# indianajohn/akaze-rust

Measured on AMD Instinct MI355X. Metric: Mpix/s through extract_features (4 oct x 4 sub), higher is better.
Workload: dtype f32

## Files before the change

### akaze-rust_amd/csrc/akz_api.cpp

```cpp
#include "akz_ctx.hpp"

unsigned akz::host_cpu_share() {
    unsigned n = std::max(1u, std::thread::hardware_concurrency());
    cpu_set_t set;
    if (sched_getaffinity(0, sizeof(set), &set) == 0) n = std::max(1, CPU_COUNT(&set));
    if (FILE* f = fopen("/sys/fs/cgroup/cpu.max", "r")) {
        char q[32] = {0};
        long period = 0;
        if (fscanf(f, "%31s %ld", q, &period) == 2 && period > 0 && strcmp(q, "max") != 0)
            n = std::min<unsigned>(n, (unsigned)std::max(1L, atol(q) / period));
        fclose(f);
    }
    if (const char* e = std::getenv("LOCAL_WORLD_SIZE")) {
        const int ranks = atoi(e);
        if (ranks > 1) n = std::max(2u, n / (unsigned)ranks);
    }
    return std::max(1u, n);
}

int level_info_out(const std::vector<LevelPlan>& plan, uint64_t level, double* etime, double* esigma,
                          uint32_t* octave, uint32_t* sublevel, uint32_t* sigma_size, uint32_t* lw, uint32_t* lh,
                          uint32_t* det_sigma, uint64_t* n_tau, double* tau, uint64_t tau_cap) {
    if (level >= plan.size()) {
        set_error("level out of range");
// ... 390 lines not shown
}
int akz_ctx_set_match_mode(akz_ctx* c, int mode) {
    AKZ_TRY(bind(c));
    if (mode < 0 || mode > 3) return AKZ_ERR_INVALID_ARG;
    c->match_mode = mode;
    for (akz_ctx* l : c->lanes) l->match_mode = mode;
    return AKZ_OK;
}
int akz_ctx_set_fed_mode(akz_ctx* c, int mode) {
    AKZ_TRY(bind(c));
    if (mode != 0 && mode != 2) return AKZ_ERR_INVALID_ARG;
    c->fed_mode = mode;
    for (akz_ctx* l : c->lanes) l->fed_mode = mode;
    return AKZ_OK;
}
const char* akz_fed_kernel_name(void) { return "k_level_march + k_fed_own"; }
int akz_debug_march_bands(int kind, uint32_t w, uint32_t h, uint32_t n, int half_width, int32_t* rows, uint32_t cap,
                          uint32_t* n_bands) {
    if (!n_bands || (cap && !rows) || kind < 0 || kind > 1 || w < 16 || h < 16 || n == 0 || half_width < 1 || half_width > 4)
        return AKZ_ERR_INVALID_ARG;
    *n_bands = launch::march_band_rows(kind, w, h, n, half_width, rows, cap);
    return AKZ_OK;
}
const char* akz_detector_kernel_name(void) { return "detector (k_detector_march + k_detector_tiled)"; }
int akz_debug_set_schedule(akz_ctx* c, int key, int value) {
    if (!c || key < 0 || key > 10) return AKZ_ERR_INVALID_ARG;
    AKZ_TRY(bind(c));
    c->sched[key] = value;
    if (key == 7 || key == 8) launch::march_min_band_rows(c->sched[7], c->sched[8]);
    if (key == 4) {
        c->big_px_sync = value > 0 ? (uint64_t)value * 1000u : gates::kBigPxSync;
        c->big_px_async = value > 0 ? (uint64_t)value * 1000u : gates::kBigPxAsync;
        c->lane_px = value > 0 ? (uint64_t)value * 1000u : gates::kLanePx;
        for (akz_ctx* l : c->lanes) {
            l->big_px_sync = std::max(c->big_px_sync, c->lane_px);
            l->big_px_async = std::max(c->big_px_async, c->lane_px);
        }
    }
    return AKZ_OK;
}
int akz_debug_placement_verdict(float spin_pair_ms, float tiny_pair_ms, float tiny_alone_ms, float spin_ms) {
    return akz::placement_verdict(spin_pair_ms, tiny_pair_ms, tiny_alone_ms, spin_ms);
}
int akz_debug_stream_placement(akz_ctx* c, int* info) {
    if (!c || !info) return AKZ_ERR_INVALID_ARG;
    AKZ_TRY(bind(c));
    info[0] = c->placed ? 1 : 0;
    info[1] = c->pre_mode;
    info[2] = c->place_replaced;
    info[3] = c->place_collisions + c->lane_collisions;
    return AKZ_OK;
}
// ... 86 lines not shown
```

### akaze-rust_amd/csrc/akz_ctx.hpp

```cpp
#pragma once
#include <algorithm>
#include <cmath>
#include <cstdlib>
#include <cstddef>
#include <cstring>
#include <atomic>
#include <condition_variable>
#include <functional>
#include <map>
#include <memory>
#include <mutex>
#include <thread>
#include <sched.h>
#include <time.h>
#include <type_traits>

#include "akz_internal.hpp"
#include "akz_select.hpp"
#include "akz_pool.hpp"
#include "akz_gates.hpp"

#define AKZ_LOCAL __attribute__((visibility("hidden")))

namespace akz {
// ... 103 lines not shown
    std::atomic<uint32_t> cand_cap_hint{1u << 15};
    std::atomic<int> live_results{0};
    bool dead = false;
    std::atomic<uint32_t> last_total_cands{0};
    std::atomic<uint64_t> last_cand_shape{0};
    hipStream_t aux = nullptr;
    std::mutex aux_m;
    hipStream_t coarse = nullptr;
    hipStream_t pre = nullptr;
    hipEvent_t pre_done = nullptr;
    hipStream_t copy = nullptr;
    DevBuf stage[kSlots];
    hipEvent_t staged[kSlots] = {nullptr, nullptr, nullptr};
    std::vector<akz_ctx*> lanes;
    unsigned next_lane = 0;
    bool is_lane = false;
    bool eager_finish = true;
    std::shared_ptr<Finisher> fin;
    hipEvent_t lane_in = nullptr;
    uint64_t stream_min_px = gates::kStreamPx;
    int prep_mode = 2;
    int det_mode = 2;
    int fed_mode = 2;
    int sched[11] = {0, 1, 0, 0, 0, 0, 0, 0, 0, 0, 0};
    uint64_t big_px = gates::kBigPxAsync;
    uint64_t big_px_sync = gates::kBigPxSync, big_px_async = gates::kBigPxAsync;
    uint64_t lane_px = gates::kLanePx;
    static constexpr uint64_t kLaunchMarchPx = gates::kMarchPx;
    uint64_t launch_min_px = kLaunchMarchPx;
    bool placed = false;
    int pre_mode = 0;
    int place_replaced = 0;
    int place_collisions = 0;
    int place_retries = 0;
    int lane_collisions = 0;
    hipEvent_t probe_ev[2] = {nullptr, nullptr};
    int profiling = 0;
    akz_profile prof{};
    struct Span { int stage; hipEvent_t a, b; int row; };
    std::vector<Span> spans;
    std::vector<akz_kernel_row> rows;
    std::vector<hipEvent_t> ev_pool;
    std::mutex ev_m;
    static constexpr int kFedRing = 4;
    hipEvent_t fed_ev[kFedRing] = {nullptr, nullptr, nullptr, nullptr};
    hipEvent_t pre_ev[kFedRing] = {nullptr, nullptr, nullptr, nullptr};
    std::atomic<uint64_t> begin_seq{0};
// ... 238 lines not shown
```

### akaze-rust_amd/csrc/akz_extract_begin.cpp

```cpp
#include "akz_extract.hpp"

namespace {
enum class Prep : uint8_t {
    Tiled,
    Stream,
    LevelMarch,
    Resident
};
enum class Det : uint8_t {
    Fallback,
    NmsFused,
    TiledSet,
    March
};
struct BeginRoute {
    bool big = false;
    int prep_mode = 0;
    int pre_on = 0;
    bool level1_clone = false;
    size_t res_first = 0;
    size_t fork_level = 0;
    size_t oct1 = 0;
    bool own_kernels = true;
    struct Level {
// ... 244 lines not shown
    StageTimer st(c, AKZ_ST_FED);
    st.kernel(AKZ_KR_FED_OWN, n_tau, lv.w, lv.h, n, fed_num_launches(c, n_tau, lv.w, lv.h, n), 0, (uint64_t)lv.w * lv.h * n * n_tau);
    AKZ_TRY(fed_impl(c, fed_in, A, B, b.P(i, AKZ_LFLOW), b.keep_all ? b.P(i, AKZ_LSTEP) : nullptr, lv.w, lv.h, n, lv.tau.data(), n_tau,
                     ride ? &np : nullptr, &rode));
    b.prepared[i + 1] = rode ? 1 : 0;
    return AKZ_OK;
}

int run_levels(BeginState& b, size_t lo, size_t hi) {
    akz_ctx* c = b.c;
    const std::vector<LevelPlan>& plan = b.r->plan;
    for (size_t i = lo; i < hi; ++i) {
        if (i >= 2) interleave_detector(b, i - 1);
        if (i == b.rt.res_first) return resident_tail(b, i);
        float* A = b.P(i, AKZ_LT);
        const bool on_coarse = i >= b.rt.fork_level;
        if (on_coarse) AKZ_TRY(ensure(c, c->scratch_coarse, plane_bytes(plan[b.rt.fork_level].w, plan[b.rt.fork_level].h, b.n)));
        float* B = (float*)(on_coarse ? c->scratch_coarse.p : c->scratch[5].p);
        AKZ_TRY(b.rt.lv[i].prep == Prep::LevelMarch ? level_by_march(b, i, A, B) : level_by_launches(b, i, A, B));
    }
    return AKZ_OK;
}

int detectors(BeginState& b, size_t lo, size_t hi, hipStream_t on) {
    akz_ctx* c = b.c;
    const akz_config& cfg = b.r->cfg;
    const uint32_t n = b.n;
    std::map<uint32_t, std::vector<launch::DetLevelDesc>> sets;
    for (size_t l = lo; l < hi; ++l) {
        if (b.det_done[l]) continue;
        const LevelPlan& lv = b.r->plan[l];
        const float thr = (float)cfg.detector_threshold, bm = border_margin(lv, cfg);
        if (b.rt.lv[l].det == Det::TiledSet) {
            sets[lv.det_sigma].push_back(launch::DetLevelDesc{b.P(l, AKZ_LSMOOTH), b.P(l, AKZ_LX), b.P(l, AKZ_LY), b.P(l, AKZ_LXX),
                                                             b.P(l, AKZ_LYY), b.P(l, AKZ_LXY), b.P(l, AKZ_LDET), lv.w, lv.h, (uint32_t)l, bm});
            continue;
        }
        if (detector_one_pass(b, l, on)) continue;
        {
            StageTimer st(c, AKZ_ST_DETECTOR);
            AKZ_TRY(detector_impl(c, b.P(l, AKZ_LSMOOTH), lv.det_sigma, b.P(l, AKZ_LX), b.P(l, AKZ_LY), b.P(l, AKZ_LXX),
                                  b.P(l, AKZ_LYY), b.P(l, AKZ_LXY), b.P(l, AKZ_LDET), lv.w, lv.h, n));
        }
        StageTimer st(c, AKZ_ST_NMS);
        launch::nms(on, b.P(l, AKZ_LDET), lv.w, lv.h, n, (uint64_t)lv.w * lv.h, (uint32_t)l, thr, bm, b.d_cand, b.cap, b.d_count);
    }
    for (auto& kv : sets) {
        const uint32_t maxn = launch::detector_tiled_set_max();
        for (size_t i = 0; i < kv.second.size(); i += maxn) {
            StageTimer st(c, AKZ_ST_DETECTOR, on);
            if (c->profiling) {
                c->prof.det_launches += 1;
                uint64_t set_px = 0;
                for (size_t j = i; j < std::min(kv.second.size(), i + maxn); ++j) set_px += (uint64_t)kv.second[j].w * kv.second[j].h * n;
                c->prof.det_px += set_px;
                st.kernel(AKZ_KR_DETECTOR_TILED, kv.first, kv.second[i].w, kv.second[i].h, n, 1, set_px);
            }
            launch::detector_tiled_set(on, kv.first, kv.second.data() + i, (uint32_t)std::min<size_t>(maxn, kv.second.size() - i),
                                       n, (float)cfg.detector_threshold, b.d_cand, b.cap, b.d_count);
        }
    }
    return AKZ_OK;
}

int fork_and_join(BeginState& b, hipStream_t* done_on) {
    akz_ctx* c = b.c;
    hipStream_t s = b.s;
    if (!c->coarse) AKZ_HIP_TRY(hipStreamCreateWithFlags(&c->coarse, hipStreamNonBlocking));
// ... 120 lines not shown
```

### akaze-rust_amd/csrc/akz_internal.hpp

```cpp
#pragma once
#include <hip/hip_runtime.h>

#include <cstdint>
#include <functional>
#include <string>
#include <vector>

#include "../../include/akaze_hip.h"
#include "../../include/akaze_hip_debug.h"

namespace akz {

void set_error(const std::string& msg);
unsigned host_cpu_share();

using TrialsOnDevice = std::function<int(const float*, const float*, const float*, const float*, uint32_t, const uint32_t*, uint32_t,
                                         float, float, float*, int32_t*)>;
int remove_outliers_impl(const akz_keypoint* keypoints_0, uint64_t n0, const akz_keypoint* keypoints_1, uint64_t n1,
                         const akz_match* matches, uint64_t n_matches, uint64_t num_trials, float epsilon_model,
                         float epsilon_inlier, akz_match* out, uint64_t* n_out, const TrialsOnDevice& trials_on_device);

#define AKZ_HIP_TRY(expr)                                                                          \
    do {                                                                                           \
        hipError_t _e = (expr);                                                                    \
// ... 163 lines not shown
                          float* lyy, float* lxy, float* ldet_out, uint32_t w, uint32_t h, uint32_t n, uint32_t level,
                          float thr, float border_m, Candidate* d_cand, uint32_t cap, uint32_t* d_count);
bool blur5_stream_supported(uint32_t w, uint32_t h, uint32_t ntaps, bool is_u8);
void blur5_stream_u8(hipStream_t s, const uint8_t* in, float* out, uint32_t w, uint32_t h, uint32_t n, const float* k);
void blur5_stream_f32(hipStream_t s, const float* in, float* out, uint32_t w, uint32_t h, uint32_t n, const float* k);
uint32_t march_band_rows(int kind, uint32_t w, uint32_t h, uint32_t n, int S, int32_t* cs_ce, uint32_t cap);
bool blur5_march_supported(uint32_t w, uint32_t h, uint32_t ntaps);
void blur5_march_u8(hipStream_t s, const uint8_t* in, float* out, uint32_t w, uint32_t h, uint32_t n, const float* k);
void blur5_march_f32(hipStream_t s, const float* in, float* out, uint32_t w, uint32_t h, uint32_t n, const float* k);
bool contrast_march_supported(uint32_t w, uint32_t h, uint32_t ntaps, uint32_t nbins);
void contrast_march(hipStream_t s, const float* in, uint32_t w, uint32_t h, uint32_t n, const float* g3,
                    unsigned long long* d_hmax_bits, uint32_t nbins, uint32_t* d_hist, double* d_thr);
void contrast_thresholds(hipStream_t s, const unsigned long long* d_hmax_bits, uint32_t nbins, uint32_t n, double* d_thr);
bool contrast_stream_supported(uint32_t w, uint32_t h, uint32_t ntaps, uint32_t nbins);
void contrast_stream(hipStream_t s, const float* in, uint32_t w, uint32_t h, uint32_t n, const float* g3,
                     unsigned long long* d_hmax_bits, uint32_t nbins, uint32_t* d_hist, double* d_thr);
bool prep_stream_supported(uint32_t w, uint32_t h);
void prep_stream(hipStream_t s, const float* prev, bool half, float* lt_out, float* lsmooth, float* lflow, uint32_t w,
                 uint32_t h, uint32_t pw, uint32_t ph, uint32_t n, const float* g3, const double* d_k, uint32_t k_pow);
bool detector_march_supported(uint32_t sigma, uint32_t w, uint32_t h, float border_m, bool nms);
void detector_march(hipStream_t s, const float* lsmooth, uint32_t sigma, float* lx, float* ly, float* lxx, float* lyy,
                    float* lxy, float* ldet_out, uint32_t w, uint32_t h, uint32_t n, uint32_t level, float thr,
                    float border_m, Candidate* d_cand, uint32_t cap, uint32_t* d_count);
bool head_fused_supported(uint32_t w, uint32_t h, uint32_t ntaps0, uint32_t ntaps1);
void head_fused_u8(hipStream_t s, const uint8_t* in, float* lt0, float* blurred, float* gx, float* gy, uint32_t w, uint32_t h, uint32_t n,
                   const float* k5, const float* g3, unsigned long long* d_smax_bits, uint32_t* d_zero_word = nullptr);
void head_fused_f32(hipStream_t s, const float* in, float* lt0, float* blurred, float* gx, float* gy, uint32_t w, uint32_t h, uint32_t n,
                    const float* k5, const float* g3, unsigned long long* d_smax_bits, uint32_t* d_zero_word = nullptr);
void contrast_hist_final(hipStream_t s, const float* gx, const float* gy, uint32_t w, uint32_t h, uint32_t n, unsigned long long* d_smax_bits,
                         uint32_t nbins, uint32_t* d_hist, uint32_t* d_done, double percentile, double* d_k);
void flow_from_pair(hipStream_t s, const float* gx, const float* gy, float* lflow, uint32_t w, uint32_t h, uint32_t n, const double* d_k,
                    uint32_t k_pow);
void march_min_band_rows(int detector, int level);
bool level_march_supported(uint32_t w, uint32_t h);
bool level_march_half_supported(uint32_t w, uint32_t h, uint32_t pw, uint32_t ph, uint32_t n_steps);
void level_march(hipStream_t s, const float* prev, float* lsmooth, float* lflow, float* lt_out, float* lstep, uint32_t w,
                 uint32_t h, uint32_t n, const float* g3, const double* d_k, uint32_t k_pow, const float* half_taus,
                 uint32_t n_steps, uint32_t pw = 0, uint32_t ph = 0);
struct ResidentLevel {
    float *lt, *lsmooth, *lflow, *lstep;
    uint32_t w, h;
    bool half;
    uint32_t n_tau;
    const float* half_tau;
    uint32_t k_pow;
};
// ... 164 lines not shown
```

### akaze-rust_amd/csrc/akz_march.hip

```cpp
#include <hip/hip_runtime.h>

#include <algorithm>
#include <cstdlib>
#include <type_traits>

#include "akz_internal.hpp"
#include "akz_pm_g2.hpp"

namespace akz {
namespace {

typedef float f2 __attribute__((ext_vector_type(2)));
typedef float f2u __attribute__((ext_vector_type(2), aligned(4)));

constexpr int MT = 256;
constexpr int MW = 2 * MT;
constexpr int HALO = 16;
constexpr int USE = MW - 2 * HALO;
constexpr int PAD = 8;
constexpr int ROW = MW + 2 * PAD;
constexpr int CBUF = 32;
#ifndef AKZ_MARCH_PF
#define AKZ_MARCH_PF 3
#endif
// ... 11 lines not shown
    return (int)((blockIdx.x & 7u) * (gridDim.x >> 3) + (blockIdx.x >> 3));
#else
    return (int)blockIdx.x;
#endif
}
__host__ __device__ __forceinline__ void uniform_band_rows(const MarchGrid& g, int band, int S, int h, int* cs, int* ce) {
    *cs = S + band * g.band_rows;
    const int e = *cs + g.band_rows;
    *ce = e < h - S ? e : h - S;
}
__host__ __device__ __forceinline__ void level_band_rows(const MarchGrid& g, int band, int h, int* cs, int* ce) {
    *cs = 1 + (band == 0 ? 0 : g.edge_rows + (band - 1) * g.band_rows);
    const int e = *cs + (band == 0 ? g.edge_rows : g.band_rows);
    *ce = band == g.nbands - 1 ? h - 1 : (e < h - 1 ? e : h - 1);
}
struct MarchNms {
    unsigned level;
    float thr;
    int xlo, xhi, ylo, yhi;
    Candidate* cand;
    unsigned cap;
    unsigned* count;
};

__device__ __forceinline__ int clampi(int v, int lo, int hi) { return v < lo ? lo : (v > hi ? hi : v); }
__device__ __forceinline__ f2 tap_main(f2 a, f2 b, f2 c, float kn, float kwn) {
    const f2 z = {0.0f, 0.0f};
    return ((z + kn * a) + kwn * b) + kn * c;
}
__device__ __forceinline__ f2 tap_off(f2 a, f2 c) {
    const f2 z = {0.0f, 0.0f};
    return (z - a) + c;
}

__device__ __forceinline__ void cands_flush(Candidate* buf, unsigned& n, const MarchNms& nms, int lane) {
    if (n == 0) return;
    unsigned base = 0;
    if (lane == 0) base = atomicAdd(nms.count, n);
    base = (unsigned)__builtin_amdgcn_readfirstlane((int)base);
    const uint4* src = reinterpret_cast<const uint4*>(buf);
    uint4* dst = reinterpret_cast<uint4*>(nms.cand);
    for (unsigned e = (unsigned)lane; e < 2u * n; e += 64u)
        if (base + (e >> 1) < nms.cap) dst[2 * (size_t)base + e] = src[e];
    __builtin_amdgcn_wave_barrier();
    n = 0;
}
// ... 89 lines not shown
            __builtin_amdgcn_raw_buffer_store_b32(__float_as_uint(a), plane[i], (int)vo0, (int)ro, AUX);
            __builtin_amdgcn_raw_buffer_store_b32(__float_as_uint(b), plane[i], (int)vo1, (int)ro, AUX);
        }
    }
}
template <int S, int N, bool ODDW, bool NT = true>
__device__ __forceinline__ void store_filled(const __amdgpu_buffer_rsrc_t (&plane)[N], const Cols& C, int w, int h, int r, bool on,
                                             const f2 (&v)[N]) {
    store_rows<N, ODDW, NT>(plane, r, w, on, C, v);
    if (on && (r == S || r == h - 1 - S)) {
        if (r == S) {
#pragma nounroll
            for (int y = 0; y < S; ++y) store_rows<N, ODDW, NT>(plane, y, w, true, C, v);
        }
        if (r == h - 1 - S) {
#pragma nounroll
            for (int y = h - S; y < h; ++y) store_rows<N, ODDW, NT>(plane, y, w, true, C, v);
        }
    }
}

template <int S, bool NMS, bool KEEP, bool ODDW>
__global__ void __launch_bounds__(MT, 3)
k_detector_march(const float* __restrict__ ls, float* __restrict__ lx_out, float* __restrict__ ly_out,
                 float* __restrict__ lxx_out, float* __restrict__ lyy_out, float* __restrict__ lxy_out,
                 float* __restrict__ ldet_out, int w, int h, MarchGrid g, float kn, float kwn, float quat, MarchNms nms) {
    constexpr int P = 2 * S + 1, NOUT = KEEP ? 4 : 1;
    static_assert(2 * S + 2 <= HALO, "strip halo");
    constexpr int R = P % 3 == 0 ? 3 : P;
    constexpr int PF = AKZ_MARCH_PF < R - 1 ? AKZ_MARCH_PF : R - 1;
    static_assert(S <= PAD, "LDS padding");
    __shared__ __attribute__((aligned(16))) float s_row[2][4][ROW];
    __shared__ Candidate s_cands[NMS ? MT / 64 : 1][NMS ? CBUF : 1];
    const int tid = threadIdx.x, lane = tid & 63;
    const int wv = __builtin_amdgcn_readfirstlane(tid >> 6);
    Candidate* const cbuf = s_cands[NMS ? wv : 0];
    unsigned cnum = 0;
    const int per = g.nbands * g.nstrips;
    const int cell = march_cell();
    if (cell >= g.total) return;
    const int img = __builtin_amdgcn_readfirstlane(cell / per);
    const int rem = cell - img * per;
    const int band = __builtin_amdgcn_readfirstlane(rem / g.nstrips), strip = rem - band * g.nstrips;
    int cs, ce;
    uniform_band_rows(g, band, S, h, &cs, &ce);
    if (cs >= ce) return;

    const int X0 = strip * USE - HALO;
    const int p0 = (2 * tid + HALO) & (MW - 1);
    const bool inner = p0 >= HALO && p0 < MW - HALO;
    const Cols C = make_cols(X0 + p0, inner, w);
    const int i0 = PAD + clampi(clampi(C.x0, S, w - 1 - S) - X0, 0, MW - 1) - S;
    const int i1 = PAD + clampi(clampi(C.x0 + 1, S, w - 1 - S) - X0, 0, MW - 1) - S;
    const int wi = PAD + p0;
    unsigned xok = 0;
    if (NMS) {
        if (inner && C.x0 < w && C.x0 >= nms.xlo && C.x0 <= nms.xhi) xok |= 1u;
        if (inner && C.x0 + 1 < w && C.x0 + 1 >= nms.xlo && C.x0 + 1 <= nms.xhi) xok |= 2u;
    }

    const size_t base = (size_t)img * (size_t)w * (size_t)h;
    const __amdgpu_buffer_rsrc_t in = plane_rsrc(ls + base, w, h);
    const __amdgpu_buffer_rsrc_t out1[2] = {plane_rsrc(lx_out + base, w, h), plane_rsrc(ly_out + base, w, h)};
    __amdgpu_buffer_rsrc_t out2[NOUT];
    out2[0] = plane_rsrc(ldet_out + base, w, h);
    if (KEEP) {
// ... 601 lines not shown
                a = f2{r0[0], r1[0]}; b = f2{r0[1], r1[1]}; m = f2{r0[2], r1[2]}; d = f2{r0[3], r1[3]}; e = f2{r0[4], r1[4]};
            }
            RH[k] = tap5(a, b, m, d, e, tp);
            const f2 o[1] = {tap5(RH[(k + 1) % P], RH[(k + 2) % P], RH[(k + 3) % P], RH[(k + 4) % P], RH[k], tp)};
            store_filled<S, 1, ODDW, false>(rout, C, w, h, c, t >= 2 * S && c >= cs && c < ce, o);
        }
    }
}

}
namespace launch {
static int g_det_min_rows = 0, g_lvl_min_rows = 0, g_head_min_rows = 0;
void march_min_band_rows(int detector, int level) {
    g_det_min_rows = detector;
    g_lvl_min_rows = level % 1000;
    g_head_min_rows = level / 1000;
}
}
namespace {
using launch::g_det_min_rows;
using launch::g_lvl_min_rows;
using launch::g_head_min_rows;

inline MarchGrid plan_level_march(uint32_t w, uint32_t h, uint32_t n, dim3* grid, int fill_wg = 3, int min_band_rows = 64) {
    static int cus = 0;
    if (!cus) {
        int dev = 0;
        hipDeviceProp_t p;
        if (hipGetDevice(&dev) == hipSuccess && hipGetDeviceProperties(&p, dev) == hipSuccess) cus = p.multiProcessorCount;
        if (cus <= 0) cus = 256;
    }
    const int fill = fill_wg, min_rows = min_band_rows;
    MarchGrid g;
    g.nstrips = (int)((w + USE - 1) / USE);
    const int rows = (int)h - 2;
    const long cols = (long)n * g.nstrips;
    const long want = ((long)cus * fill + cols - 1) / cols;
    long nb = std::max<long>(1, std::min<long>(want, std::max(1, rows / min_rows)));
    constexpr int edge_pct = 75;
    if (nb >= 3) {
        const double m = (double)rows / ((double)(nb - 2) + 2.0 * edge_pct / 100.0);
        g.band_rows = std::max(1, (int)(m + 0.999));
        g.edge_rows = std::max(1, (int)((rows - (long)(nb - 2) * g.band_rows) / 2));
        g.nbands = (int)nb;
        if (g.edge_rows + (long)(nb - 2) * g.band_rows >= rows) {
            g.band_rows = (int)((rows + nb - 1) / nb);
            g.edge_rows = g.band_rows;
            g.nbands = (rows + g.band_rows - 1) / g.band_rows;
        }
    } else {
        g.band_rows = (int)((rows + nb - 1) / nb);
        g.edge_rows = g.band_rows;
        g.nbands = (rows + g.band_rows - 1) / g.band_rows;
    }
    g.total = (int)(cols * g.nbands);
    *grid = dim3((unsigned)((g.total + 7) / 8 * 8));
    return g;
}

inline MarchGrid plan_march(uint32_t w, uint32_t h, uint32_t n, int S, dim3* grid, int fill_wg = 3, int min_band_rows = 64) {
    static int cus = 0;
    if (!cus) {
        int dev = 0;
        hipDeviceProp_t p;
        if (hipGetDevice(&dev) == hipSuccess && hipGetDeviceProperties(&p, dev) == hipSuccess) cus = p.multiProcessorCount;
        if (cus <= 0) cus = 256;
    }
    const int fill = fill_wg, min_rows = min_band_rows;
    const int use = USE;
    (void)S;
    MarchGrid g;
    g.nstrips = (int)((w + use - 1) / use);
    const int rows = (int)h - 2 * S;
    const long cols = (long)n * g.nstrips;
    const long want = ((long)cus * fill + cols - 1) / cols;
    long nb = std::max<long>(1, std::min<long>(want, std::max(1, rows / min_rows)));
    g.band_rows = (int)((rows + nb - 1) / nb);
    g.edge_rows = g.band_rows;
    g.nbands = (rows + g.band_rows - 1) / g.band_rows;
    g.total = (int)(cols * g.nbands);
    *grid = dim3((unsigned)((g.total + 7) / 8 * 8));
    return g;
}

}

namespace launch {

static void admissible_range(uint32_t dim, float border_m, int* lo, int* hi) {
    auto out_lo = [&](int v) { return (roundf((float)v - border_m) - 1.0f) < 0.0f; };
    auto out_hi = [&](int v) { return (roundf((float)v + border_m) + 1.0f) >= (float)dim; };
    int a = 1, b = (int)dim - 2;
    while (a <= b && out_lo(a)) ++a;
    while (b >= a && out_hi(b)) --b;
    *lo = a;
    *hi = b;
}

bool detector_march_supported(uint32_t sigma, uint32_t w, uint32_t h, float border_m, bool nms) {
    if (sigma < 1 || sigma > 4) return false;
    if (w < 4 * sigma + 8 || h < 4 * sigma + 8) return false;
    if ((uint64_t)w * h > (1ull << 28)) return false;
    return !nms || border_m >= (float)(sigma + 2);
}


template <int S, bool NMS, bool KEEP>
static void launch_detector_march(hipStream_t s, const float* lsmooth, float* lx, float* ly, float* lxx, float* lyy, float* lxy,
                                  float* ldet_out, uint32_t w, uint32_t h, uint32_t n, float kn, float kwn, float quat,
                                  const MarchNms& na) {
    dim3 gr;
#ifndef AKZ_DET_FILL
#define AKZ_DET_FILL 3
#endif
#ifndef AKZ_DET_MINROWS
#define AKZ_DET_MINROWS 40
#endif
    const int few_cols_rows = (uint64_t)n * ((w + USE - 1) / USE) <= 4 ? 24 : AKZ_DET_MINROWS;
    const MarchGrid mg = plan_march(w, h, n, S, &gr, AKZ_DET_FILL, g_det_min_rows > 0 ? g_det_min_rows : few_cols_rows);
    if (w & 1u)
        hipLaunchKernelGGL((k_detector_march<S, NMS, KEEP, true>), gr, dim3(MT), 0, s, lsmooth, lx, ly, lxx, lyy, lxy, ldet_out,
                           (int)w, (int)h, mg, kn, kwn, quat, na);
    else
        hipLaunchKernelGGL((k_detector_march<S, NMS, KEEP, false>), gr, dim3(MT), 0, s, lsmooth, lx, ly, lxx, lyy, lxy, ldet_out,
                           (int)w, (int)h, mg, kn, kwn, quat, na);
}
#define AKZ_MARCH(S)                                                                                              \
    case S: {                                                                                                     \
        if (d_cand && keep)                                                                                       \
            launch_detector_march<S, true, true>(s, lsmooth, lx, ly, lxx, lyy, lxy, ldet_out, w, h, n, kn, kwn, quat, na);   \
        else if (d_cand)                                                                                          \
            launch_detector_march<S, true, false>(s, lsmooth, lx, ly, lxx, lyy, lxy, ldet_out, w, h, n, kn, kwn, quat, na);  \
        else if (keep)                                                                                            \
            launch_detector_march<S, false, true>(s, lsmooth, lx, ly, lxx, lyy, lxy, ldet_out, w, h, n, kn, kwn, quat, na);  \
        else                                                                                                      \
            launch_detector_march<S, false, false>(s, lsmooth, lx, ly, lxx, lyy, lxy, ldet_out, w, h, n, kn, kwn, quat, na); \
    } break;

void detector_march(hipStream_t s, const float* lsmooth, uint32_t sigma, float* lx, float* ly, float* lxx, float* lyy,
                    float* lxy, float* ldet_out, uint32_t w, uint32_t h, uint32_t n, uint32_t level, float thr,
                    float border_m, Candidate* d_cand, uint32_t cap, uint32_t* d_count) {
    const Taps m = taps_scharr_main(sigma);
    const float kn = m.wgt[0], kwn = m.wgt[1];
    const float quat = (float)(sigma * sigma * sigma * sigma);
    const bool keep = lxx && lyy && lxy;
    MarchNms na{level, thr, 0, -1, 0, -1, d_cand, cap, d_count};
    if (d_cand) {
        admissible_range(w, border_m, &na.xlo, &na.xhi);
        admissible_range(h, border_m, &na.ylo, &na.yhi);
    }
    switch (sigma) {
        AKZ_MARCH(1) AKZ_MARCH(2) AKZ_MARCH(3) AKZ_MARCH(4)
        default: break;
    }
}
#undef AKZ_MARCH

bool blur5_march_supported(uint32_t w, uint32_t h, uint32_t ntaps) {
    return ntaps == 5 && w >= 16 && h >= 16 && (uint64_t)w * h <= (1ull << 28);
}
template <typename T>
static void blur5_march_t(hipStream_t s, const T* in, float* out, uint32_t w, uint32_t h, uint32_t n, const float* k) {
    BlurTaps5 tp;
    for (int i = 0; i < 5; ++i) tp.k[i] = k[i];
    dim3 gr;
    const MarchGrid mg = plan_march(w, h, n, 2, &gr, 6, g_head_min_rows > 0 ? g_head_min_rows : 32);
    if (w & 1u) hipLaunchKernelGGL((k_blur5_march<T, true>), gr, dim3(MT), 0, s, in, out, (int)w, (int)h, mg, tp);
    else hipLaunchKernelGGL((k_blur5_march<T, false>), gr, dim3(MT), 0, s, in, out, (int)w, (int)h, mg, tp);
}
void blur5_march_u8(hipStream_t s, const uint8_t* in, float* out, uint32_t w, uint32_t h, uint32_t n, const float* k) {
    blur5_march_t<uint8_t>(s, in, out, w, h, n, k);
}
void blur5_march_f32(hipStream_t s, const float* in, float* out, uint32_t w, uint32_t h, uint32_t n, const float* k) {
    blur5_march_t<float>(s, in, out, w, h, n, k);
}

bool contrast_march_supported(uint32_t w, uint32_t h, uint32_t ntaps, uint32_t nbins) {
    return ntaps == 3 && nbins >= 1 && nbins <= 640 && level_march_supported(w, h);
}
// ... 85 lines not shown
```

### akaze-rust_amd/python/akaze_amd.py

```python
import ctypes as C
import os

import numpy as np

_PKG = os.path.dirname(os.path.dirname(os.path.abspath(__file__)))
LIB_PATH = os.environ.get("AKAZE_HIP_LIB") or os.path.join(_PKG, "libakaze_hip.so")

AKZ_KEEP_ALL_PLANES = 1
AKZ_NO_HOST_DESCRIPTORS = 2
AKZ_NO_DETECT = 4
AKZ_INPUT_READY = 8
AKZ_ERR_BUFFER = -7

PLANES = ["Lt", "Lsmooth", "Lx", "Ly", "Lxx", "Lyy", "Lxy", "Lflow", "Lstep", "Ldet"]


class AkazeError(RuntimeError):
    def __init__(self, status, msg):
        super().__init__(f"akaze_hip status {status}: {msg}")
        self.status = status


class Config(C.Structure):
    _fields_ = [
# ... 169 lines not shown
        "akz_result_counts": ([vp, u64, pu64, pu64, pu64], i32),
        "akz_result_keypoints": ([vp, u64, vp], i32),
        "akz_result_descriptors": ([vp, u64, vp], i32),
        "akz_result_device_descriptors": ([vp, u64, C.POINTER(vp), pu64], i32),
        "akz_result_contrast": ([vp, u64, pf64], i32),
        "akz_result_copy_device_descriptors": ([vp, vp, u64, pu64], i32),
        "akz_result_level_info": ([vp, u64, pf64, pf64, pu32, pu32, pu32, pu32, pu32, pu64, pf64, u64], i32),
        "akz_fetch_plane": ([vp, u64, u64, i32, vp, pu64], i32),
        "akz_fetch_pyramid": ([vp, u64, vp, u64, pu64], i32),
        "akz_result_device_plane": ([vp, u64, u64, i32, C.POINTER(vp)], i32),
        "akz_descriptor_match": ([vp, vp, u64, vp, u64, u64, u64, f64, vp, pu64], i32),
        "akz_descriptor_match_device": ([vp, vp, u64, vp, u64, u64, f64, vp, vp], i32),
        "akz_ctx_graph_probe": ([vp, vp, u32, u32, u32, C.POINTER(Config), u32, u32, pf64, pf64, pu64], i32),
        "akz_debug_march_bands": ([i32, u32, u32, u32, i32, C.POINTER(i32), u32, pu32], i32),
        "akz_ctx_set_lanes": ([vp, u32], i32),
        "akz_ctx_set_eager_finish": ([vp, i32], i32),
        "akz_fed_kernel_name": ([], C.c_char_p),
        "akz_ctx_set_host_threads": ([vp, u32], i32),
        "akz_debug_set_match_chunks": ([vp, u32, u32], i32),
        "akz_debug_set_host_sort": ([vp, i32], i32),
        "akz_debug_set_select": ([vp, i32], i32),
        "akz_debug_select_info": ([vp, C.POINTER(C.c_int)], i32),
        "akz_debug_set_schedule": ([vp, i32, i32], i32),
        "akz_debug_stream_placement": ([vp, C.POINTER(i32)], i32),
        "akz_detector_kernel_name": ([], C.c_char_p),
        "akz_remove_outliers": ([vp, u64, vp, u64, vp, u64, u64, C.c_float, C.c_float, vp, pu64], i32),
        "akz_estimate_fundamental_matrix": ([vp, u64, vp, u64, vp, C.c_float, fp, C.POINTER(i32)], i32),
        "akz_match_features": ([vp, vp, u64, vp, u64, vp, u64, vp, u64, u64, f64, u64, C.c_float, vp, pu64], i32),
        "akz_match_features_pairs": ([vp, vp, u64, vp, u64, u64, f64, u64, C.c_float, vp, pu64], i32),
        "akz_debug_ransac_samples": ([u64, u64, u64, u64, pu64], i32),
        "akz_debug_ransac_samples_k": ([u64, u64, u64, u64, i32, pu64], i32),
        "akz_estimate_homography": ([vp, u64, vp, u64, vp, C.c_float, fp, C.POINTER(i32)], i32),
        "akz_remove_outliers_homography": ([vp, u64, vp, u64, vp, u64, u64, C.c_float, C.c_float, vp, pu64, fp, C.POINTER(i32)], i32),
        "akz_match_features_homography": ([vp, vp, u64, vp, u64, vp, u64, vp, u64, u64, f64, u64, C.c_float, vp, pu64, fp,
                                           C.POINTER(i32)], i32),
        "akz_match_features_homography_pairs": ([vp, vp, u64, vp, u64, u64, f64, u64, C.c_float, vp, pu64, fp, C.POINTER(i32)], i32),
        "akz_refine_homography": ([vp, u64, vp, u64, vp, u64, fp, C.c_float, C.c_uint32, vp, pu64, fp, C.POINTER(C.c_uint32)], i32),
        "akz_match_features_homography_refined": ([vp, vp, u64, vp, u64, vp, u64, vp, u64, u64, f64, u64, C.c_float, C.c_uint32, vp, pu64,
                                                   fp, C.POINTER(i32), C.POINTER(C.c_uint32)], i32),
        "akz_match_features_homography_refined_pairs": ([vp, vp, u64, vp, u64, u64, f64, u64, C.c_float, C.c_uint32, vp, pu64, fp,
                                                         C.POINTER(i32), C.POINTER(C.c_uint32)], i32),
        "akz_match_features_homography_refined_guided": ([vp, vp, u64, vp, u64, vp, u64, vp, u64, u64, f64, u64, C.c_float, C.c_uint32,
                                                          C.c_float, f64, vp, pu64, fp, C.POINTER(i32), C.POINTER(C.c_uint32)], i32),
        "akz_match_features_homography_refined_guided_pairs": ([vp, vp, u64, vp, u64, u64, f64, u64, C.c_float, C.c_uint32, C.c_float, f64,
                                                                vp, pu64, fp, C.POINTER(i32), C.POINTER(C.c_uint32)], i32),
        "akz_descriptor_match_guided_host": ([vp, u64, vp, u64, vp, u64, vp, u64, u64, i32, fp, C.c_float, u64, f64, vp, pu64], i32),
# ... 1751 lines not shown
```

### include/akaze_hip_debug.h

```cpp
#ifndef AKAZE_HIP_DEBUG_H
#define AKAZE_HIP_DEBUG_H
#include "akaze_hip.h"
#ifdef __cplusplus
extern "C" {
#endif

int akz_ctx_graph_probe(akz_ctx* ctx, const uint8_t* d_imgs, uint32_t w, uint32_t h, uint32_t n, const akz_config* cfg,
                        uint32_t flags, uint32_t reps, double* ms_graph, double* ms_plain, uint64_t* graph_nodes);
int akz_debug_march_bands(int kind, uint32_t w, uint32_t h, uint32_t n, int half_width, int32_t* rows, uint32_t cap,
                          uint32_t* n_bands);
const char* akz_fed_kernel_name(void);
const char* akz_detector_kernel_name(void);
int akz_debug_set_match_chunks(akz_ctx* ctx, uint32_t pair_chunks, uint32_t set_chunks);
int akz_debug_match_tile_rows(uint32_t* rows);
int akz_debug_set_schedule(akz_ctx* ctx, int key, int value);
int akz_debug_stream_placement(akz_ctx* ctx, int* info);
int akz_debug_placement_verdict(float spin_pair_ms, float tiny_pair_ms, float tiny_alone_ms, float spin_ms);
int akz_debug_device_libm(akz_ctx* ctx, int* available, int* last_job);
int akz_debug_set_device_libm(akz_ctx* ctx, int mode);
int akz_debug_libm_eval(akz_ctx* ctx, const float* d_a, const float* d_b, float* d_out3, uint64_t n, int fma);
typedef struct akz_gate {
    const char* name;
    double value;
    const char* unit;
    const char* meaning;
} akz_gate;
int akz_debug_gates(const akz_gate** rows, uint64_t* n);
int akz_ctx_calibrate_gates(akz_ctx* ctx, uint64_t* sync_px, uint64_t* async_px, double* ms);
enum { AKZ_KR_LEVEL_MARCH = 1, AKZ_KR_FED_OWN = 2, AKZ_KR_OCTAVE_RESIDENT = 3, AKZ_KR_DETECTOR_TILED = 4, AKZ_KR_DETECTOR_MARCH = 5,
       AKZ_KR_JPEG_IDCT = 6, AKZ_KR_JPEG_LUMA = 7, AKZ_KR_JPEG_COPY = 8 };
typedef struct akz_kernel_row {
    uint32_t stage, kind, param, w, h, n;
    uint64_t launches, px, px_steps;
// ... 24 lines not shown
```

Measured before the change: 14610.

## Batch march-detector levels of equal sigma into one multi-level launch

Levels that use the march detector and share a detector sigma and width parity are grouped and launched as one kernel. Each workgroup decodes which level, image, band and strip it owns from a per-launch table of up to four entries. Band counts are planned jointly across the grouped levels so the combined grid targets a fixed number of waves over the CUs. This removes per-level launch overhead and the tail underfill of small coarse levels, at the cost of extra per-block indexing, larger kernel arguments, and less flexible per-level band sizing.

```diff
diff --git a/akaze-rust_amd/csrc/akz_api.cpp b/akaze-rust_amd/csrc/akz_api.cpp
--- a/akaze-rust_amd/csrc/akz_api.cpp
+++ b/akaze-rust_amd/csrc/akz_api.cpp
@@ -436,12 +436,23 @@
     *n_bands = launch::march_band_rows(kind, w, h, n, half_width, rows, cap);
     return AKZ_OK;
 }
+int akz_debug_detector_set_cells(int half_width, const uint32_t* w, const uint32_t* h, uint32_t n_entries, uint32_t n, int32_t* cells,
+                                 uint32_t cap, int32_t* grids, uint32_t* n_workgroups) {
+    if (!n_workgroups || !w || !h || !grids || (cap && !cells) || n_entries < 1 || n_entries > launch::detector_march_set_max() || n == 0 ||
+        half_width < 1 || half_width > 4)
+        return AKZ_ERR_INVALID_ARG;
+    for (uint32_t e = 0; e < n_entries; ++e)
+        if (w[e] < 4u * (uint32_t)half_width + 8u || h[e] < 4u * (uint32_t)half_width + 8u) return AKZ_ERR_INVALID_ARG;
+    *n_workgroups = launch::detector_set_cells(half_width, w, h, n_entries, n, cells, cap, grids);
+    return AKZ_OK;
+}
 const char* akz_detector_kernel_name(void) { return "detector (k_detector_march + k_detector_tiled)"; }
 int akz_debug_set_schedule(akz_ctx* c, int key, int value) {
-    if (!c || key < 0 || key > 10) return AKZ_ERR_INVALID_ARG;
+    if (!c || key < 0 || key > 11) return AKZ_ERR_INVALID_ARG;
     AKZ_TRY(bind(c));
     c->sched[key] = value;
     if (key == 7 || key == 8) launch::march_min_band_rows(c->sched[7], c->sched[8]);
+    if (key == 11) launch::detector_set_waves(value >= 11 && value <= 14 ? value - 10 : 0);
     if (key == 4) {
         c->big_px_sync = value > 0 ? (uint64_t)value * 1000u : gates::kBigPxSync;
         c->big_px_async = value > 0 ? (uint64_t)value * 1000u : gates::kBigPxAsync;
diff --git a/akaze-rust_amd/csrc/akz_ctx.hpp b/akaze-rust_amd/csrc/akz_ctx.hpp
--- a/akaze-rust_amd/csrc/akz_ctx.hpp
+++ b/akaze-rust_amd/csrc/akz_ctx.hpp
@@ -149,7 +149,7 @@
     int prep_mode = 2;
     int det_mode = 2;
     int fed_mode = 2;
-    int sched[11] = {0, 1, 0, 0, 0, 0, 0, 0, 0, 0, 0};
+    int sched[12] = {0, 1, 0, 0, 0, 0, 0, 0, 0, 0, 0, 0};
     uint64_t big_px = gates::kBigPxAsync;
     uint64_t big_px_sync = gates::kBigPxSync, big_px_async = gates::kBigPxAsync;
     uint64_t lane_px = gates::kLanePx;
diff --git a/akaze-rust_amd/csrc/akz_extract_begin.cpp b/akaze-rust_amd/csrc/akz_extract_begin.cpp
--- a/akaze-rust_amd/csrc/akz_extract_begin.cpp
+++ b/akaze-rust_amd/csrc/akz_extract_begin.cpp
@@ -290,15 +290,23 @@
     return AKZ_OK;
 }
 
+constexpr bool kDetSetsByDefault = true;
 int detectors(BeginState& b, size_t lo, size_t hi, hipStream_t on) {
     akz_ctx* c = b.c;
     const akz_config& cfg = b.r->cfg;
     const uint32_t n = b.n;
     std::map<uint32_t, std::vector<launch::DetLevelDesc>> sets;
+    std::map<std::pair<uint32_t, uint32_t>, std::vector<launch::DetLevelDesc>> march_sets;
+    const bool by_sets = c->sched[11] == 0 ? kDetSetsByDefault : c->sched[11] != 1;
     for (size_t l = lo; l < hi; ++l) {
         if (b.det_done[l]) continue;
         const LevelPlan& lv = b.r->plan[l];
         const float thr = (float)cfg.detector_threshold, bm = border_margin(lv, cfg);
+        if (by_sets && b.rt.lv[l].det == Det::March) {
+            march_sets[{lv.det_sigma, lv.w & 1u}].push_back(launch::DetLevelDesc{b.P(l, AKZ_LSMOOTH), b.P(l, AKZ_LX), b.P(l, AKZ_LY), b.P(l, AKZ_LXX),
+                                                                                 b.P(l, AKZ_LYY), b.P(l, AKZ_LXY), b.P(l, AKZ_LDET), lv.w, lv.h, (uint32_t)l, bm});
+            continue;
+        }
         if (b.rt.lv[l].det == Det::TiledSet) {
             sets[lv.det_sigma].push_back(launch::DetLevelDesc{b.P(l, AKZ_LSMOOTH), b.P(l, AKZ_LX), b.P(l, AKZ_LY), b.P(l, AKZ_LXX),
                                                              b.P(l, AKZ_LYY), b.P(l, AKZ_LXY), b.P(l, AKZ_LDET), lv.w, lv.h, (uint32_t)l, bm});
@@ -312,6 +320,23 @@
         }
         StageTimer st(c, AKZ_ST_NMS);
         launch::nms(on, b.P(l, AKZ_LDET), lv.w, lv.h, n, (uint64_t)lv.w * lv.h, (uint32_t)l, thr, bm, b.d_cand, b.cap, b.d_count);
+    }
+    for (auto& kv : march_sets) {
+        std::vector<launch::DetLevelDesc>& v = kv.second;
+        std::stable_sort(v.begin(), v.end(), [](const launch::DetLevelDesc& x, const launch::DetLevelDesc& y) { return (uint64_t)x.w * x.h > (uint64_t)y.w * y.h; });
+        const uint32_t maxn = launch::detector_march_set_max();
+        for (size_t i = 0; i < v.size(); i += maxn) {
+            const uint32_t cnt = (uint32_t)std::min<size_t>(maxn, v.size() - i);
+            StageTimer st(c, AKZ_ST_DETECTOR, on);
+            if (c->profiling) {
+                c->prof.det_launches += 1;
+                uint64_t set_px = 0;
+                for (size_t j = i; j < i + cnt; ++j) set_px += (uint64_t)v[j].w * v[j].h * n;
+                c->prof.det_px += set_px;
+                st.kernel(AKZ_KR_DETECTOR_MARCH, kv.first.first, v[i].w, v[i].h, n, 1, set_px);
+            }
+            launch::detector_march_set(on, kv.first.first, v.data() + i, cnt, n, (float)cfg.detector_threshold, b.d_cand, b.cap, b.d_count);
+        }
     }
     for (auto& kv : sets) {
         const uint32_t maxn = launch::detector_tiled_set_max();
diff --git a/akaze-rust_amd/csrc/akz_internal.hpp b/akaze-rust_amd/csrc/akz_internal.hpp
--- a/akaze-rust_amd/csrc/akz_internal.hpp
+++ b/akaze-rust_amd/csrc/akz_internal.hpp
@@ -209,6 +209,12 @@
 void detector_march(hipStream_t s, const float* lsmooth, uint32_t sigma, float* lx, float* ly, float* lxx, float* lyy,
                     float* lxy, float* ldet_out, uint32_t w, uint32_t h, uint32_t n, uint32_t level, float thr,
                     float border_m, Candidate* d_cand, uint32_t cap, uint32_t* d_count);
+uint32_t detector_march_set_max();
+void detector_march_set(hipStream_t s, uint32_t sigma, const DetLevelDesc* levels, uint32_t nlevels, uint32_t n, float thr,
+                        Candidate* d_cand, uint32_t cap, uint32_t* d_count);
+void detector_set_waves(int waves);
+uint32_t detector_set_cells(int S, const uint32_t* w, const uint32_t* h, uint32_t nlv, uint32_t n, int32_t* cells, uint32_t cap,
+                            int32_t* grids);
 bool head_fused_supported(uint32_t w, uint32_t h, uint32_t ntaps0, uint32_t ntaps1);
 void head_fused_u8(hipStream_t s, const uint8_t* in, float* lt0, float* blurred, float* gx, float* gy, uint32_t w, uint32_t h, uint32_t n,
                    const float* k5, const float* g3, unsigned long long* d_smax_bits, uint32_t* d_zero_word = nullptr);
diff --git a/akaze-rust_amd/csrc/akz_march.hip b/akaze-rust_amd/csrc/akz_march.hip
--- a/akaze-rust_amd/csrc/akz_march.hip
+++ b/akaze-rust_amd/csrc/akz_march.hip
@@ -57,6 +57,53 @@
     unsigned cap;
     unsigned* count;
 };
+
+constexpr int kDetSetMax = 4;
+struct DetMarchEntry {
+    const float* ls;
+    float *lx, *ly, *ldet, *lxx, *lyy, *lxy;
+    int w, h;
+    MarchGrid g;
+    unsigned level;
+    int xlo, xhi, ylo, yhi;
+    int first;
+};
+struct DetMarchSet {
+    DetMarchEntry e[kDetSetMax];
+};
+#if defined(__HIP_DEVICE_COMPILE__)
+#define AKZ_UNIFORM(x) __builtin_amdgcn_readfirstlane(x)
+#else
+#define AKZ_UNIFORM(x) (x)
+#endif
+__host__ __device__ __forceinline__ bool det_set_cell(const DetMarchSet& set, int wg, int nwg, DetMarchEntry* E, int* entry, int* img,
+                                                      int* band, int* strip) {
+#if AKZ_MARCH_XCD
+    const int xcd = wg & 7, j = wg >> 3;
+    (void)nwg;
+#else
+    const int xcd = wg / (nwg >> 3), j = wg - xcd * (nwg >> 3);
+#endif
+    DetMarchEntry X = set.e[0];
+    int e = 0, jl = j;
+    const int f1 = set.e[1].first, f2 = set.e[2].first, f3 = set.e[3].first;
+    if (j >= f1) { X = set.e[1]; e = 1; jl = j - f1; }
+    if (j >= f2) { X = set.e[2]; e = 2; jl = j - f2; }
+    if (j >= f3) { X = set.e[3]; e = 3; jl = j - f3; }
+    static_assert(kDetSetMax == 4, "compare chain");
+    const int cell = AKZ_UNIFORM(xcd * ((X.g.total + 7) >> 3) + jl);
+    if (cell >= X.g.total) return false;
+    const int per = X.g.nbands * X.g.nstrips;
+    const int i = AKZ_UNIFORM(cell / per);
+    const int rem = cell - i * per;
+    const int b = AKZ_UNIFORM(rem / X.g.nstrips);
+    *E = X;
+    *entry = e;
+    *img = i;
+    *band = b;
+    *strip = rem - b * X.g.nstrips;
+    return true;
+}
 
 __device__ __forceinline__ int clampi(int v, int lo, int hi) { return v < lo ? lo : (v > hi ? hi : v); }
 __device__ __forceinline__ f2 tap_main(f2 a, f2 b, f2 c, float kn, float kwn) {
@@ -192,9 +239,8 @@
 
 template <int S, bool NMS, bool KEEP, bool ODDW>
 __global__ void __launch_bounds__(MT, 3)
-k_detector_march(const float* __restrict__ ls, float* __restrict__ lx_out, float* __restrict__ ly_out,
-                 float* __restrict__ lxx_out, float* __restrict__ lyy_out, float* __restrict__ lxy_out,
-                 float* __restrict__ ldet_out, int w, int h, MarchGrid g, float kn, float kwn, float quat, MarchNms nms) {
+k_detector_march(DetMarchSet set, float kn, float kwn, float quat, float thr, Candidate* __restrict__ cand, unsigned cap,
+                 unsigned* __restrict__ count) {
     constexpr int P = 2 * S + 1, NOUT = KEEP ? 4 : 1;
     static_assert(2 * S + 2 <= HALO, "strip halo");
     constexpr int R = P % 3 == 0 ? 3 : P;
@@ -206,12 +252,19 @@
     const int wv = __builtin_amdgcn_readfirstlane(tid >> 6);
     Candidate* const cbuf = s_cands[NMS ? wv : 0];
     unsigned cnum = 0;
-    const int per = g.nbands * g.nstrips;
-    const int cell = march_cell();
-    if (cell >= g.total) return;
-    const int img = __builtin_amdgcn_readfirstlane(cell / per);
-    const int rem = cell - img * per;
-    const int band = __builtin_amdgcn_readfirstlane(rem / g.nstrips), strip = rem - band * g.nstrips;
+    DetMarchEntry E;
+    int entry, img, band, strip;
+    if (!det_set_cell(set, (int)blockIdx.x, (int)gridDim.x, &E, &entry, &img, &band, &strip)) return;
+    const float* __restrict__ const ls = E.ls;
+    float* __restrict__ const lx_out = E.lx;
+    float* __restrict__ const ly_out = E.ly;
+    float* __restrict__ const lxx_out = E.lxx;
+    float* __restrict__ const lyy_out = E.lyy;
+    float* __restrict__ const lxy_out = E.lxy;
+    float* __restrict__ const ldet_out = E.ldet;
+    const int w = E.w, h = E.h;
+    const MarchGrid g = E.g;
+    const MarchNms nms{E.level, thr, E.xlo, E.xhi, E.ylo, E.yhi, cand, cap, count};
     int cs, ce;
     uniform_band_rows(g, band, S, h, &cs, &ce);
     if (cs >= ce) return;
@@ -859,7 +912,7 @@
 using launch::g_lvl_min_rows;
 using launch::g_head_min_rows;
 
-inline MarchGrid plan_level_march(uint32_t w, uint32_t h, uint32_t n, dim3* grid, int fill_wg = 3, int min_band_rows = 64) {
+inline int march_cus() {
     static int cus = 0;
     if (!cus) {
         int dev = 0;
@@ -867,6 +920,10 @@
         if (hipGetDevice(&dev) == hipSuccess && hipGetDeviceProperties(&p, dev) == hipSuccess) cus = p.multiProcessorCount;
         if (cus <= 0) cus = 256;
     }
+    return cus;
+}
+inline MarchGrid plan_level_march(uint32_t w, uint32_t h, uint32_t n, dim3* grid, int fill_wg = 3, int min_band_rows = 64) {
+    const int cus = march_cus();
     const int fill = fill_wg, min_rows = min_band_rows;
     MarchGrid g;
     g.nstrips = (int)((w + USE - 1) / USE);
@@ -896,13 +953,7 @@
 }
 
 inline MarchGrid plan_march(uint32_t w, uint32_t h, uint32_t n, int S, dim3* grid, int fill_wg = 3, int min_band_rows = 64) {
-    static int cus = 0;
-    if (!cus) {
-        int dev = 0;
-        hipDeviceProp_t p;
-        if (hipGetDevice(&dev) == hipSuccess && hipGetDeviceProperties(&p, dev) == hipSuccess) cus = p.multiProcessorCount;
-        if (cus <= 0) cus = 256;
-    }
+    const int cus = march_cus();
     const int fill = fill_wg, min_rows = min_band_rows;
     const int use = USE;
     (void)S;
@@ -942,56 +993,128 @@
 }
 
 
-template <int S, bool NMS, bool KEEP>
-static void launch_detector_march(hipStream_t s, const float* lsmooth, float* lx, float* ly, float* lxx, float* lyy, float* lxy,
-                                  float* ldet_out, uint32_t w, uint32_t h, uint32_t n, float kn, float kwn, float quat,
-                                  const MarchNms& na) {
-    dim3 gr;
 #ifndef AKZ_DET_FILL
 #define AKZ_DET_FILL 3
 #endif
 #ifndef AKZ_DET_MINROWS
 #define AKZ_DET_MINROWS 40
 #endif
-    const int few_cols_rows = (uint64_t)n * ((w + USE - 1) / USE) <= 4 ? 24 : AKZ_DET_MINROWS;
-    const MarchGrid mg = plan_march(w, h, n, S, &gr, AKZ_DET_FILL, g_det_min_rows > 0 ? g_det_min_rows : few_cols_rows);
-    if (w & 1u)
-        hipLaunchKernelGGL((k_detector_march<S, NMS, KEEP, true>), gr, dim3(MT), 0, s, lsmooth, lx, ly, lxx, lyy, lxy, ldet_out,
-                           (int)w, (int)h, mg, kn, kwn, quat, na);
+static int det_min_band_rows(uint32_t w, uint32_t n) {
+    if (g_det_min_rows > 0) return g_det_min_rows;
+    return (uint64_t)n * ((w + USE - 1) / USE) <= 4 ? 24 : AKZ_DET_MINROWS;
+}
+constexpr int kDetSetWaves = 1;
+static int g_det_set_waves = 0;
+void detector_set_waves(int waves) { g_det_set_waves = waves >= 1 && waves <= 4 ? waves : 0; }
+
+static void plan_march_set(const DetLevelDesc* lv, uint32_t nlv, uint32_t n, int S, MarchGrid* grids) {
+    if (nlv == 1) {
+        dim3 gr;
+        grids[0] = plan_march(lv[0].w, lv[0].h, n, S, &gr, AKZ_DET_FILL, det_min_band_rows(lv[0].w, n));
+        return;
+    }
+    uint64_t strip_rows = 0;
+    for (uint32_t e = 0; e < nlv; ++e) strip_rows += (uint64_t)n * ((lv[e].w + USE - 1) / USE) * (lv[e].h - 2 * (uint32_t)S);
+    const uint64_t target = (uint64_t)march_cus() * AKZ_DET_FILL * (uint64_t)(g_det_set_waves ? g_det_set_waves : kDetSetWaves);
+    for (uint32_t e = 0; e < nlv; ++e) {
+        MarchGrid g;
+        g.nstrips = (int)((lv[e].w + USE - 1) / USE);
+        const long rows = (long)lv[e].h - 2 * S;
+        const long want = (long)((target * (uint64_t)rows + strip_rows - 1) / strip_rows);
+        const long nb = std::max<long>(1, std::min<long>(want, std::max<long>(1, rows / det_min_band_rows(lv[e].w, n))));
+        g.band_rows = (int)((rows + nb - 1) / nb);
+        g.edge_rows = g.band_rows;
+        g.nbands = (int)((rows + g.band_rows - 1) / g.band_rows);
+        g.total = (int)((long)n * g.nstrips * g.nbands);
+        grids[e] = g;
+    }
+}
+static unsigned make_det_set(const DetLevelDesc* lv, uint32_t nlv, uint32_t n, int S, bool nms, DetMarchSet* set) {
+    MarchGrid grids[kDetSetMax];
+    plan_march_set(lv, nlv, n, S, grids);
+    int first = 0;
+    for (uint32_t e = 0; e < (uint32_t)kDetSetMax; ++e) {
+        DetMarchEntry& E = set->e[e];
+        if (e >= nlv) {
+            E = DetMarchEntry{};
+            E.first = 0x7fffffff;
+            continue;
+        }
+        E = DetMarchEntry{lv[e].lsmooth, lv[e].lx, lv[e].ly, lv[e].ldet, lv[e].lxx, lv[e].lyy, lv[e].lxy, (int)lv[e].w, (int)lv[e].h,
+                          grids[e], lv[e].level, 0, -1, 0, -1, first};
+        if (nms) {
+            admissible_range(lv[e].w, lv[e].border_m, &E.xlo, &E.xhi);
+            admissible_range(lv[e].h, lv[e].border_m, &E.ylo, &E.yhi);
+        }
+        first += (grids[e].total + 7) / 8;
+    }
+    return (unsigned)first * 8u;
+}
+
+template <int S, bool NMS, bool KEEP>
+static void launch_detector_march(hipStream_t s, const DetMarchSet& set, unsigned nwg, bool oddw, float kn, float kwn, float quat, float thr,
+                                  Candidate* d_cand, uint32_t cap, uint32_t* d_count) {
+    if (oddw)
+        hipLaunchKernelGGL((k_detector_march<S, NMS, KEEP, true>), dim3(nwg), dim3(MT), 0, s, set, kn, kwn, quat, thr, d_cand, cap, d_count);
     else
-        hipLaunchKernelGGL((k_detector_march<S, NMS, KEEP, false>), gr, dim3(MT), 0, s, lsmooth, lx, ly, lxx, lyy, lxy, ldet_out,
-                           (int)w, (int)h, mg, kn, kwn, quat, na);
-}
-#define AKZ_MARCH(S)                                                                                              \
-    case S: {                                                                                                     \
-        if (d_cand && keep)                                                                                       \
-            launch_detector_march<S, true, true>(s, lsmooth, lx, ly, lxx, lyy, lxy, ldet_out, w, h, n, kn, kwn, quat, na);   \
-        else if (d_cand)                                                                                          \
-            launch_detector_march<S, true, false>(s, lsmooth, lx, ly, lxx, lyy, lxy, ldet_out, w, h, n, kn, kwn, quat, na);  \
-        else if (keep)                                                                                            \
-            launch_detector_march<S, false, true>(s, lsmooth, lx, ly, lxx, lyy, lxy, ldet_out, w, h, n, kn, kwn, quat, na);  \
-        else                                                                                                      \
-            launch_detector_march<S, false, false>(s, lsmooth, lx, ly, lxx, lyy, lxy, ldet_out, w, h, n, kn, kwn, quat, na); \
+        hipLaunchKernelGGL((k_detector_march<S, NMS, KEEP, false>), dim3(nwg), dim3(MT), 0, s, set, kn, kwn, quat, thr, d_cand, cap, d_count);
+}
+#define AKZ_MARCH(S)                                                                                               \
+    case S: {                                                                                                      \
+        const unsigned nwg = make_det_set(levels, nlevels, n, S, d_cand != nullptr, &set);                         \
+        if (d_cand && keep) launch_detector_march<S, true, true>(s, set, nwg, oddw, kn, kwn, quat, thr, d_cand, cap, d_count);    \
+        else if (d_cand) launch_detector_march<S, true, false>(s, set, nwg, oddw, kn, kwn, quat, thr, d_cand, cap, d_count);      \
+        else if (keep) launch_detector_march<S, false, true>(s, set, nwg, oddw, kn, kwn, quat, thr, d_cand, cap, d_count);        \
+        else launch_detector_march<S, false, false>(s, set, nwg, oddw, kn, kwn, quat, thr, d_cand, cap, d_count);                 \
     } break;
 
+uint32_t detector_march_set_max() { return (uint32_t)kDetSetMax; }
+void detector_march_set(hipStream_t s, uint32_t sigma, const DetLevelDesc* levels, uint32_t nlevels, uint32_t n, float thr,
+                        Candidate* d_cand, uint32_t cap, uint32_t* d_count) {
+    if (nlevels == 0 || nlevels > (uint32_t)kDetSetMax) return;
+    const Taps m = taps_scharr_main(sigma);
+    const float kn = m.wgt[0], kwn = m.wgt[1];
+    const float quat = (float)(sigma * sigma * sigma * sigma);
+    const bool keep = levels[0].lxx && levels[0].lyy && levels[0].lxy;
+    const bool oddw = (levels[0].w & 1u) != 0;
+    DetMarchSet set;
+    switch (sigma) {
+        AKZ_MARCH(1) AKZ_MARCH(2) AKZ_MARCH(3) AKZ_MARCH(4)
+        default: break;
+    }
+}
+#undef AKZ_MARCH
 void detector_march(hipStream_t s, const float* lsmooth, uint32_t sigma, float* lx, float* ly, float* lxx, float* lyy,
                     float* lxy, float* ldet_out, uint32_t w, uint32_t h, uint32_t n, uint32_t level, float thr,
                     float border_m, Candidate* d_cand, uint32_t cap, uint32_t* d_count) {
-    const Taps m = taps_scharr_main(sigma);
-    const float kn = m.wgt[0], kwn = m.wgt[1];
-    const float quat = (float)(sigma * sigma * sigma * sigma);
-    const bool keep = lxx && lyy && lxy;
-    MarchNms na{level, thr, 0, -1, 0, -1, d_cand, cap, d_count};
-    if (d_cand) {
-        admissible_range(w, border_m, &na.xlo, &na.xhi);
-        admissible_range(h, border_m, &na.ylo, &na.yhi);
-    }
-    switch (sigma) {
-        AKZ_MARCH(1) AKZ_MARCH(2) AKZ_MARCH(3) AKZ_MARCH(4)
-        default: break;
-    }
-}
-#undef AKZ_MARCH
+    const DetLevelDesc one{lsmooth, lx, ly, lxx, lyy, lxy, ldet_out, w, h, level, border_m};
+    detector_march_set(s, sigma, &one, 1, n, thr, d_cand, cap, d_count);
+}
+uint32_t detector_set_cells(int S, const uint32_t* w, const uint32_t* h, uint32_t nlv, uint32_t n, int32_t* cells, uint32_t cap,
+                            int32_t* grids) {
+    DetLevelDesc lv[kDetSetMax] = {};
+    for (uint32_t e = 0; e < nlv; ++e) {
+        lv[e].w = w[e];
+        lv[e].h = h[e];
+    }
+    DetMarchSet set;
+    const unsigned nwg = make_det_set(lv, nlv, n, S, false, &set);
+    for (uint32_t e = 0; e < nlv; ++e) {
+        grids[3 * e] = set.e[e].g.nstrips;
+        grids[3 * e + 1] = set.e[e].g.nbands;
+        grids[3 * e + 2] = set.e[e].g.band_rows;
+    }
+    for (unsigned i = 0; i < nwg && i < cap; ++i) {
+        DetMarchEntry E;
+        int entry = -1, img = -1, band = -1, strip = -1;
+        if (!det_set_cell(set, (int)i, (int)nwg, &E, &entry, &img, &band, &strip)) entry = img = band = strip = -1;
+        cells[4 * i] = entry;
+        cells[4 * i + 1] = img;
+        cells[4 * i + 2] = band;
+        cells[4 * i + 3] = strip;
+    }
+    return nwg;
+}
 
 bool blur5_march_supported(uint32_t w, uint32_t h, uint32_t ntaps) {
     return ntaps == 5 && w >= 16 && h >= 16 && (uint64_t)w * h <= (1ull << 28);
diff --git a/akaze-rust_amd/python/akaze_amd.py b/akaze-rust_amd/python/akaze_amd.py
--- a/akaze-rust_amd/python/akaze_amd.py
+++ b/akaze-rust_amd/python/akaze_amd.py
@@ -215,6 +215,7 @@
         "akz_debug_set_select": ([vp, i32], i32),
         "akz_debug_select_info": ([vp, C.POINTER(C.c_int)], i32),
         "akz_debug_set_schedule": ([vp, i32, i32], i32),
+        "akz_debug_detector_set_cells": ([i32, pu32, pu32, u32, u32, C.POINTER(i32), u32, C.POINTER(i32), pu32], i32),
         "akz_debug_stream_placement": ([vp, C.POINTER(i32)], i32),
         "akz_detector_kernel_name": ([], C.c_char_p),
         "akz_remove_outliers": ([vp, u64, vp, u64, vp, u64, u64, C.c_float, C.c_float, vp, pu64], i32),
diff --git a/include/akaze_hip_debug.h b/include/akaze_hip_debug.h
--- a/include/akaze_hip_debug.h
+++ b/include/akaze_hip_debug.h
@@ -9,6 +9,8 @@
                         uint32_t flags, uint32_t reps, double* ms_graph, double* ms_plain, uint64_t* graph_nodes);
 int akz_debug_march_bands(int kind, uint32_t w, uint32_t h, uint32_t n, int half_width, int32_t* rows, uint32_t cap,
                           uint32_t* n_bands);
+int akz_debug_detector_set_cells(int half_width, const uint32_t* w, const uint32_t* h, uint32_t n_entries, uint32_t n, int32_t* cells,
+                                 uint32_t cap, int32_t* grids, uint32_t* n_workgroups);
 const char* akz_fed_kernel_name(void);
 const char* akz_detector_kernel_name(void);
 int akz_debug_set_match_chunks(akz_ctx* ctx, uint32_t pair_chunks, uint32_t set_chunks);
```

New measurement: 14910 (median of 6 runs). 1.02x the previous value.
